# bmds-lab/Crackling

Measured on AMD Instinct MI355X. Metric: guides/sec (whole node) + achieved HBM GB/s, 20bp/<=4mm ISSL scan, higher is better.
Workload: dtype u32

## Files before the change

### crackling_amd/csrc/issl_device.hpp

```cpp
#pragma once
#include <cstddef>
#include <cstdint>
#include <string>

#include "issl_host.hpp"

namespace issl {

constexpr uint64_t kImageMagic = 0x314C535349444D41ull;
constexpr uint32_t kImageVersion = 9;
constexpr uint32_t kTileCands = 2048;
constexpr uint32_t kHeaderBytes = 4096;

struct ImageHeader {
    uint64_t magic;
    uint32_t version;
    uint32_t kind;
    uint64_t n_sites, seq_len, n_lines, slice_width, n_slices, n_scores_file;
    uint64_t n_buckets;
    uint64_t n_scores_unique;
    uint64_t n_tiles;
    uint64_t tile_cands;
    uint64_t total_bytes;
    uint64_t off_bucket_start, off_tile_first, off_score_mask, off_score_val, off_sites, off_entries,
        off_scan;
    uint64_t off_mit_dense;
    uint64_t off_esig;
    uint64_t cold_on_host;
    uint64_t cold_bytes;
    uint64_t off_occ8;
    uint64_t off_sub_start;
    uint64_t off_srec;
    uint64_t off_sid;
    uint64_t off_site_occ;
    uint64_t lists_absent;
};
static_assert(sizeof(ImageHeader) <= kHeaderBytes, "header must fit its block");

constexpr uint32_t kOccSaturated = 0xFFFFFFu;
constexpr uint64_t kSigMask = (1ull << 40) - 1ull;

#if defined(__HIPCC__)
__host__ __device__
#endif
inline uint32_t succ_byte(uint64_t sig, uint32_t s, uint32_t slice_width)
{
    const uint32_t sh = (slice_width * (s + 1u)) % 40u;
    const uint64_t x = sig & kSigMask;
    return static_cast<uint32_t>(sh ? (x >> sh) | (x << (40u - sh)) : x) & 0xFFu;
}
struct alignas(16) StreamRec {
    uint64_t sig;
    uint32_t id;
    uint32_t pos;
};

struct ImageView {
    const uint64_t *bucket_start;
    const uint32_t *tile_first;
    const uint64_t *score_mask;
    const double *score_val;
    const double *mit_dense;
    const uint64_t *sites;
    const uint64_t *entries;
    const uint64_t *esig;
    const uint8_t *occ8;
    const uint32_t *sub_start;
    const StreamRec *srec;
    const uint32_t *sid;
    const uint32_t *site_occ;
    const uint32_t *scan;
    uint64_t n_sites;
    uint32_t n_buckets;
    uint32_t n_scores;
    uint32_t slice_width;
    uint32_t n_slices;
    uint32_t n_tiles;
};

struct LayoutSpec {
    bool inline_sigs = false;
    uint32_t cold = 0;
    uint32_t sorted = 0;
    bool no_lists = false;
};
void layout_image(ImageHeader &h, const Geometry &g, uint64_t n_scores_unique, uint64_t n_tiles, bool dense_mit,
                  const LayoutSpec &spec);
ImageView make_view(const ImageHeader &h, void *base, void *cold);

struct Tuning {
    uint32_t scan_blocks;
    uint32_t scan_threads;
    int upload_threads;
    size_t upload_chunk_kib, upload_ring_min_kib;
    uint32_t item_guides;
    bool scan_generic;
    int scan_events;
    bool stage_timing;
    bool upload_timing;
    size_t raw_chunks;
    int inline_sigs;
    int sorted_layout;
    int compact;
    int prune;
    int tail_shapes;
    int hit_slots;
    size_t fine_items;
    size_t expect_guides;
    int small_bin;
    int lean_tail;
    int lanes;
    int host_cold;
    int keep_lists;
    std::string stamps_path;
    static Tuning from_env();
    bool set(const char *key, const char *value);
    bool get(const char *key, long long *value) const;
    int set_list(const char *options);
};
bool image_option(const ImageHeader *h, const char *key, long long *value);

int launch_build_entries(const uint64_t *d_sites, const uint32_t *d_occ, uint64_t n_sites, uint32_t slice_begin,
                         uint32_t slice_end, uint32_t slice_width, uint64_t *d_entries);
int launch_bucket_sizes(const uint64_t *d_sites, uint64_t n_sites, uint32_t slice_width, uint32_t n_slices, uint64_t *h_sizes);

constexpr int kSortNeedsListOrder = -1000;
constexpr int kSortNoRoom = -1001;
struct SortTemp {
    uint64_t *keys = nullptr, *tmp = nullptr;
    uint32_t *hist = nullptr;
    bool keys_borrowed = false;
    int alloc(uint64_t n_sites, void *borrowed_keys = nullptr);
    void release();
    ~SortTemp() { release(); }
};
int launch_sort_slice(SortTemp &t, const uint64_t *d_sites, const uint64_t *d_list, const uint64_t *d_bucket_start,
                      const uint32_t *d_tile_first, uint64_t n_sites, uint32_t n_slices, uint32_t n_buckets, uint32_t slice_width, uint32_t slice, uint32_t *d_sub_start,
                      StreamRec *d_srec, uint32_t *d_sid, uint32_t *d_site_occ, uint32_t *d_flag);
int finish_sort(uint32_t *d_flag);
void launch_tag_sites(uint64_t *d_sites, const uint32_t *d_site_occ, uint64_t n_sites);

constexpr uint32_t kGuideGroup = 8;
constexpr uint32_t kItemGuides = 512;
constexpr uint32_t kGuideCost = 4;
constexpr uint32_t kTileFixedCost = 8 * kGuideCost;
constexpr uint32_t kNoGuide = 0xFFFFFFFFu;
constexpr uint32_t kPadGuideWord = 0xFFFFFFFFu;
constexpr uint32_t kScanGridBlocks = 256u * 4u;
constexpr uint32_t kScanMaxBlocks = 8192u;
constexpr uint32_t kScanWaves = kScanMaxBlocks * 16u;
constexpr uint32_t kMaxRanges = kScanMaxBlocks;
constexpr uint32_t kStampsScanWords = 4u * kScanWaves, kStampsPerReplay = 16u * 4096u;
constexpr uint32_t kStampsMid = kStampsScanWords, kStampsBig256 = kStampsMid + kStampsPerReplay, kStampsBig1024 = kStampsBig256 + kStampsPerReplay;
constexpr uint32_t kStampsWords = kStampsBig1024 + kStampsPerReplay;
constexpr uint32_t kSpanRing = 64;
constexpr uint32_t kChunkRecs = 128;
constexpr uint64_t kDeadKey = ~0ull;
constexpr uint32_t kKeySliceShift = 32, kKeyGuideShift = 37, kKeySliceMask = 31, kMaxSlices = 20;

struct ScanItem {
    uint32_t bucket;
    uint32_t g0, g1;
    uint32_t n_tiles;
    uint64_t cost0;
    uint32_t tile0;
    uint32_t last_cands;
    uint32_t group_abs;
    uint32_t window;
    uint32_t shape;
    uint32_t gmid;
};
static_assert(sizeof(ScanItem) == 48, "scan items are fetched with scalar loads");

struct RangeStart {
    uint32_t item;
    uint32_t tile;
    uint32_t goff;
    uint32_t pad;
};

struct PlanInfo {
    uint32_t n_items;
    uint32_t error;
    uint32_t n_ranges;
    uint32_t fine;
    uint64_t total_cost;
    uint64_t candidates;
    uint64_t reference_candidates;
    uint64_t tiles;
    uint32_t fine_slots;
    uint32_t pad;
};

struct Counters {
    uint32_t next_range;
    uint32_t n_big;
    uint32_t n_big2;
    uint32_t n_big3;
    uint32_t raw_chunks;
    uint32_t raw_overflow;
    uint32_t overflowed;
    uint32_t replay_next[3];
};

struct FineSum {
    uint64_t cost, cand;
    uint32_t slots, items, units;
    uint32_t places;
};

constexpr uint32_t kSlotHits = 512;
constexpr uint32_t kSlotHitsWide = 2048;
struct alignas(32) SlotRec {
    double mit, cfd;
    uint64_t key, pad;
};
#if defined(__HIPCC__)
__host__ __device__
#endif
inline uint64_t slot_pad(uint32_t occ, uint32_t dist) { return static_cast<uint64_t>(occ) | (static_cast<uint64_t>(dist) << 32); }
constexpr uint32_t kFineWays = 13;
constexpr uint32_t kFineWays2 = 67;
constexpr uint32_t kFetchPairs = 8;
constexpr uint32_t kPruneMaxGuides = 1u << 20;
constexpr uint32_t kPruneMaxGuides2 = 1u << 18;
inline uint32_t prune_max_guides(uint32_t prune_mode, uint32_t n_slices)
{
    const uint32_t m = prune_mode == 3 ? kPruneMaxGuides2 : kPruneMaxGuides;
    return n_slices > 10 ? m >> 2 : n_slices > 5 ? m >> 1 : m;
}

struct alignas(16) FineMeta {
    uint32_t guide;
    uint32_t where;
    uint64_t gsig;
};

struct Workspace {
    uint32_t *ng = nullptr;
    uint32_t *gfill = nullptr;
    uint32_t *gstart = nullptr;
    uint32_t *gword = nullptr;
    uint32_t *gidx = nullptr;
    uint32_t *gbucket = nullptr;
    ScanItem *items = nullptr;
    uint32_t *fword = nullptr;
    FineMeta *fmeta = nullptr;
    ScanItem *fitems = nullptr;
    uint32_t *fcount = nullptr;
    uint32_t *fcount0 = nullptr;
    FineSum *fsum = nullptr;
    size_t cap_fslots = 0, cap_fitems = 0;
    uint32_t fine_ways = 0;
    PlanInfo *plan = nullptr;
    RangeStart *range_start = nullptr;
    uint64_t *raw = nullptr;
    uint32_t *raw_used = nullptr;
    size_t cap_chunks = 0;
    Counters *counters = nullptr;
    unsigned long long *scan_span = nullptr;
    uint32_t span_slot = 0;
    uint64_t *scan_count = nullptr;
// ... 59 lines not shown
```

### crackling_amd/csrc/issl_kernels.hip

```cpp
#include <hip/hip_runtime.h>

#include <algorithm>
#include <type_traits>
#include <cstdio>

#include "issl_device.hpp"

namespace issl {

#define ISSL_CFD_QUAL __constant__
#include "cfd_tables.inc"


__device__ __forceinline__ void short_kernel_priority() { __builtin_amdgcn_s_setprio(3); }

__host__ __device__ inline uint32_t gather_even16(uint32_t x)
{
    x &= 0x55555555u;
    x = (x | (x >> 1)) & 0x33333333u;
    x = (x | (x >> 2)) & 0x0F0F0F0Fu;
    x = (x | (x >> 4)) & 0x00FF00FFu;
    x = (x | (x >> 8)) & 0x0000FFFFu;
    return x;
}
// ... 405 lines not shown
           (u.rest ? static_cast<uint64_t>(len) * (u.shape >> 3) + kTileFixedCost : 0ull);
}

__device__ __forceinline__ uint32_t fine_way(uint32_t gj, uint32_t way)
{
    if (way == 0) return gj;
    if (way < kFineWays) {
        const uint32_t q = (way - 1u) / 3u, d = (way - 1u) % 3u + 1u;
        return gj ^ (d << (2u * q));
    }
    const uint32_t w2 = way - kFineWays, pair = w2 / 9u, d1 = (w2 % 9u) / 3u + 1u, d2 = w2 % 3u + 1u;
    const uint32_t a = pair < 3u ? 0u : pair < 5u ? 1u : 2u;
    const uint32_t b = pair < 3u ? pair + 1u : pair < 5u ? pair - 1u : 3u;
    return gj ^ (d1 << (2u * a)) ^ (d2 << (2u * b));
}
__device__ __forceinline__ uint32_t fine_class(uint32_t way) { return way == 0u ? 0u : way < kFineWays ? 1u : 2u; }

__host__ __device__ __forceinline__ uint32_t fine_quad(uint32_t slice) { return slice < 4u ? slice : 0u; }
__host__ __device__ __forceinline__ uint32_t fine_order(uint32_t slice, uint32_t j, uint32_t slice_width = 8u)
{
    if (slice_width != 8u) return j + 1u;
    const uint32_t sq = fine_quad(slice);
    if (slice == 0u) return j + 1u;
    const uint32_t prev = slice - 1u;
    if (j == 0u) return prev;
    uint32_t q = 0, seen = 0;
    for (; q < 4u; ++q) {
        if (q == sq || q == prev) continue;
        if (++seen == j) break;
    }
    return q;
}
__host__ __device__ __forceinline__ uint32_t fine_word(uint32_t word, uint32_t slice, uint32_t slice_width = 8u)
{
    const uint32_t lo = word & 0xFFFFu, hi = word >> 16;
    uint32_t lo12 = 0, hi12 = 0;
    for (uint32_t j = 0; j < 3u; ++j) {
        const uint32_t q = fine_order(slice, j, slice_width);
        lo12 |= ((lo >> (4u * q)) & 0xFu) << (4u * j);
        hi12 |= ((hi >> (4u * q)) & 0xFu) << (4u * j);
    }
    return lo12 | (hi12 << 12);
}

template <uint32_t WAYS>
__global__ __launch_bounds__(256) void k_fine_count(ImageView v, const uint64_t *__restrict__ guides,
                                                    const uint32_t *__restrict__ gstart, const uint32_t *__restrict__ gfill,
                                                    const uint32_t *__restrict__ gidx, uint32_t *__restrict__ fcount,
                                                    uint32_t *__restrict__ fcount0,
                                                    FineSum *__restrict__ fsum, uint32_t item_guides, uint32_t tail_shapes)
{
    constexpr uint32_t ways = WAYS;
    short_kernel_priority();
    __shared__ uint32_t cnt[256], cnt0[256];
    __shared__ uint64_t lds[256];
    const uint32_t b = blockIdx.x, slice = b >> v.slice_width;
    cnt[threadIdx.x] = 0;
    cnt0[threadIdx.x] = 0;
    __syncthreads();
    const uint32_t g0 = gstart[b], n = gfill[b];
    for (uint32_t i = threadIdx.x; i < n; i += 256) {
        const uint32_t gj = succ_byte(guides[gidx[g0 + i]], slice, v.slice_width);
        atomicAdd(&cnt0[gj], 1u);
#pragma unroll
        for (uint32_t way = 0; way < ways; ++way) atomicAdd(&cnt[fine_way(gj, way)], 1u);
    }
    __syncthreads();
    const uint32_t w = threadIdx.x, c = cnt[w];
    const uint32_t *ss = v.sub_start + static_cast<uint64_t>(b) * 257u;
    const uint32_t s0 = ss[w], s1 = ss[w + 1];
    fcount[static_cast<uint64_t>(b) * 256u + w] = (s1 > s0) ? c : 0u;
    fcount0[static_cast<uint64_t>(b) * 256u + w] = (s1 > s0) ? cnt0[w] : 0u;
    uint64_t cost = 0, cand = 0, slots = 0, items = 0, units = 0;
    if (c && s1 > s0) {
        const GroupUnits gu = group_units(s0, s1, tail_shapes);
        const uint32_t kk = (c + item_guides - 1u) / item_guides;
        slots = (c + kGuideGroup - 1u) / kGuideGroup * kGuideGroup;
        units = static_cast<uint64_t>(gu.units) * kk;
        items = units;
        for (uint32_t done = 0; done < c; done += item_guides) cost += group_cost(gu, c - done < item_guides ? c - done : item_guides);
        cand = static_cast<uint64_t>(s1 - s0) * c;
    }
    uint64_t t_cost, t_cand, t_slots, t_items, t_units, t_places;
    (void)block_exclusive_scan(cost, lds, &t_cost);
    (void)block_exclusive_scan(cand, lds, &t_cand);
    (void)block_exclusive_scan(slots, lds, &t_slots);
    (void)block_exclusive_scan(items, lds, &t_items);
    (void)block_exclusive_scan(units, lds, &t_units);
    (void)block_exclusive_scan((c && s1 > s0) ? c : 0u, lds, &t_places);
    if (threadIdx.x == 0) {
        FineSum f;
        f.cost = t_cost; f.cand = t_cand; f.slots = static_cast<uint32_t>(t_slots); f.items = static_cast<uint32_t>(t_items);
        f.units = static_cast<uint32_t>(t_units); f.places = static_cast<uint32_t>(t_places);
        fsum[b] = f;
    }
}

__global__ __launch_bounds__(256) void k_fine_plan(FineSum *__restrict__ fsum, uint32_t nb, ScanItem *__restrict__ fitems,
                                                   uint32_t cap_items, uint32_t cap_slots, PlanInfo *__restrict__ plan,
                                                   uint32_t scan_blocks, uint32_t prune_mode, uint32_t always,
                                                   uint32_t *__restrict__ sticky, Counters *__restrict__ counters)
{
    short_kernel_priority();
    __shared__ uint64_t lds[256];
    const uint32_t per = (nb + 255u) / 256u;
    const uint32_t b0 = threadIdx.x * per, b1 = (b0 + per < nb) ? b0 + per : nb;
    uint64_t cost = 0, cand = 0, slots = 0, items = 0, units = 0, places = 0;
    for (uint32_t b = b0; b < b1; ++b) {
        cost += fsum[b].cost; cand += fsum[b].cand; slots += fsum[b].slots; items += fsum[b].items; units += fsum[b].units;
        places += fsum[b].places;
    }
    uint64_t t_cost, t_cand, t_slots, t_items, t_units, t_places;
    (void)block_exclusive_scan(places, lds, &t_places);
    uint64_t cost_at = block_exclusive_scan(cost, lds, &t_cost);
    (void)block_exclusive_scan(cand, lds, &t_cand);
    uint64_t slot_at = block_exclusive_scan(slots, lds, &t_slots);
    uint64_t item_at = block_exclusive_scan(items, lds, &t_items);
    uint64_t unit_at = block_exclusive_scan(units, lds, &t_units);
    for (uint32_t b = b0; b < b1; ++b) {
        const FineSum f = fsum[b];
        FineSum at;
        at.cost = cost_at; at.cand = 0; at.slots = static_cast<uint32_t>(slot_at); at.items = static_cast<uint32_t>(item_at);
        at.units = static_cast<uint32_t>(unit_at); at.places = 0;
        fsum[b] = at;
        cost_at += f.cost; slot_at += f.slots; item_at += f.items; unit_at += f.units;
    }
    if (threadIdx.x == 255) {
        const uint64_t fetch_cost = static_cast<uint64_t>(kFetchPairs) * kGuideCost;
        const uint64_t full_fetch = plan->tiles, full_pairs = plan->total_cost - kTileFixedCost * full_fetch;
        const uint64_t fine_pairs = t_cost - kTileFixedCost * t_units;
        const uint64_t est_full = full_pairs > fetch_cost * full_fetch ? full_pairs : fetch_cost * full_fetch;
        const uint64_t est_fine = (fine_pairs > fetch_cost * t_units ? fine_pairs : fetch_cost * t_units) + t_places * kGuideCost;
        const bool fits = t_items <= cap_items && t_slots <= cap_slots;
        if (t_items > cap_items)
            atomicMax(&sticky[3], static_cast<uint32_t>(t_items < 0xFFFFFFFFull ? t_items : 0xFFFFFFFFull));
        if (fits && plan->error == 0 && (always || est_fine < est_full)) {
            ScanItem end;
            end.bucket = 0; end.g0 = 0; end.g1 = 0; end.n_tiles = 0; end.cost0 = t_cost;
            end.tile0 = static_cast<uint32_t>(t_units); end.last_cands = 0; end.group_abs = 0; end.window = 0;
            end.shape = 32; end.gmid = 0;
            fitems[t_items] = end;
            plan->n_items = static_cast<uint32_t>(t_items);
            plan->total_cost = t_cost;
            plan->candidates = t_cand;
            plan->tiles = t_units;
            plan->n_ranges = t_units == 0 ? 0u : ranges_for(t_units, scan_blocks);
            counters->raw_chunks = (plan->n_ranges ? plan->n_ranges : 1u) * 16u;
            plan->fine = prune_mode;
            plan->fine_slots = static_cast<uint32_t>(t_slots);
        }
    }
}

template <uint32_t WAYS>
__global__ __launch_bounds__(256) void k_fine_scatter(ImageView v, const uint64_t *__restrict__ guides,
                                                      const uint32_t *__restrict__ gstart, const uint32_t *__restrict__ gfill,
                                                      const uint32_t *__restrict__ gword, const uint32_t *__restrict__ gidx,
                                                      const uint32_t *__restrict__ fcount, const uint32_t *__restrict__ fcount0,
                                                      const FineSum *__restrict__ fbase,
                                                      const PlanInfo *__restrict__ plan, uint32_t *__restrict__ fword,
                                                      FineMeta *__restrict__ fmeta,
                                                      ScanItem *__restrict__ fitems, uint32_t item_guides, uint32_t tail_shapes)
{
    constexpr uint32_t ways = WAYS;
    short_kernel_priority();
    if (!plan->fine) return;
    __shared__ uint64_t lds[256];
    __shared__ uint32_t slot_of[256], slot0_of[256], cursor[256], cursor0[256], has_cands[256];
    const uint32_t b = blockIdx.x, slice = b >> v.slice_width;
    const uint32_t w = threadIdx.x;
    const uint32_t c = fcount[static_cast<uint64_t>(b) * 256u + w];
    const uint32_t c1 = c - fcount0[static_cast<uint64_t>(b) * 256u + w];
    const uint32_t *ss = v.sub_start + static_cast<uint64_t>(b) * 257u;
    const uint32_t s0 = ss[w], s1 = ss[w + 1];
    uint64_t cost = 0, slots = 0, items = 0;
    uint32_t kk = 0;
    GroupUnits gu{};
    if (c) {
        gu = group_units(s0, s1, tail_shapes);
        kk = (c + item_guides - 1u) / item_guides;
        slots = (c + kGuideGroup - 1u) / kGuideGroup * kGuideGroup;
        items = static_cast<uint64_t>(gu.units) * kk;
        for (uint32_t done = 0; done < c; done += item_guides) cost += group_cost(gu, c - done < item_guides ? c - done : item_guides);
    }
    const FineSum base = fbase[b];
    uint64_t cost_at = base.cost + block_exclusive_scan(cost, lds, nullptr);
    const uint32_t slot_at = base.slots + static_cast<uint32_t>(block_exclusive_scan(slots, lds, nullptr));
    uint32_t item_at = base.items + static_cast<uint32_t>(block_exclusive_scan(items, lds, nullptr));
    slot_of[w] = slot_at;
    slot0_of[w] = slot_at + c1;
    cursor[w] = 0;
    cursor0[w] = 0;
    __shared__ uint32_t item0_of[257], c_of[256];
    __shared__ uint64_t cost0_of[256];
    __shared__ __attribute__((aligned(16))) ScanItem stage[256];
    item0_of[w] = item_at - base.items;
    if (w == 255u) item0_of[256] = item_at - base.items + static_cast<uint32_t>(items);
    c_of[w] = c;
    cost0_of[w] = cost_at;
    if (c)
        for (uint32_t k2 = c; k2 < static_cast<uint32_t>(slots); ++k2) { fmeta[slot_at + k2] = FineMeta{kNoGuide, 0u, 0ull}; fword[slot_at + k2] = kPadGuideWord; }
    has_cands[w] = s1 > s0 ? 1u : 0u;
    __syncthreads();
    {
        const uint32_t total = item0_of[256];
        const uint64_t blen = v.bucket_start[b + 1] - v.bucket_start[b];
        const uint32_t tile_first_b = v.tile_first[b];
        for (uint32_t i0 = 0; i0 < total; i0 += 256u) {
            const uint32_t i = i0 + w;
            if (i < total) {
                uint32_t lo = 0, hi = 256;
                while (hi - lo > 1u) {
                    const uint32_t mid = (lo + hi) >> 1;
                    if (item0_of[mid] <= i) lo = mid; else hi = mid;
                }
                const uint32_t gw = lo, gc = c_of[gw];
                const uint32_t gs0 = ss[gw], gs1 = ss[gw + 1];
                const GroupUnits g2 = group_units(gs0, gs1, tail_shapes);
                const uint32_t j = i - item0_of[gw];
                const uint32_t chunk = j / g2.units, t = j - chunk * g2.units;
                const uint32_t done = chunk * item_guides;
                const uint32_t len = (gc - done < item_guides) ? gc - done : item_guides;
                const bool full = t < g2.n_full;
                const uint32_t shape = full ? 32u : g2.shape, cap = 64u * shape;
                const uint32_t wstart = g2.s0a + t * kTileCands;
                const uint64_t after = blen - wstart;
                const uint32_t gslot = slot_of[gw];
                ScanItem it;
                it.bucket = (b << 8) | gw;
                it.g0 = gslot + done;
                it.g1 = it.g0 + len;
                it.n_tiles = 1;
                it.cost0 = cost0_of[gw] + static_cast<uint64_t>(chunk) * group_cost(g2, item_guides) +
                           static_cast<uint64_t>(t) * (static_cast<uint64_t>(len) * kGuideCost + kTileFixedCost);
                it.tile0 = base.items + i;
                it.last_cands = after < cap ? static_cast<uint32_t>(after) : cap;
                it.group_abs = tile_first_b * 64u + (wstart >> 5);
                it.window = (t == 0 ? gs0 - g2.s0a : 0u) | ((gs1 - wstart < cap ? gs1 - wstart : cap) << 16);
                it.shape = shape; it.gmid = slot0_of[gw];
                stage[w] = it;
            }
            __syncthreads();
            const uint32_t n_here = total - i0 < 256u ? total - i0 : 256u;
            const uint4 *src4 = reinterpret_cast<const uint4 *>(stage);
            uint4 *dst4 = reinterpret_cast<uint4 *>(fitems + base.items + i0);
            for (uint32_t q = w; q < n_here * 3u; q += 256u) dst4[q] = src4[q];
            __syncthreads();
        }
    }
    const uint32_t g0 = gstart[b], n = gfill[b];
    for (uint32_t i = threadIdx.x; i < n; i += 256) {
        const uint32_t guide = gidx[g0 + i], word = gword[g0 + i];
        const uint64_t gsig = guides[guide];
        const uint32_t gj = succ_byte(gsig, slice, v.slice_width);
        const uint32_t word12 = fine_word(word, slice, v.slice_width);
#pragma unroll
        for (uint32_t way = 0; way < ways; ++way) {
            const uint32_t ww = fine_way(gj, way);
            if (!has_cands[ww]) continue;
            const uint32_t slot = way ? slot_of[ww] + atomicAdd(&cursor[ww], 1u) : slot0_of[ww] + atomicAdd(&cursor0[ww], 1u);
            fword[slot] = word12 | (fine_class(way) << 24);
            fmeta[slot] = FineMeta{guide, (b << 8) | ww, gsig};
        }
    }
}

__global__ __launch_bounds__(256) void k_fine_ranges(const PlanInfo *__restrict__ plan, const ScanItem *__restrict__ fitems,
                                                     RangeStart *__restrict__ starts)
{
    short_kernel_priority();
    if (!plan->fine) return;
    const uint32_t n_ranges = plan->n_ranges;
    const uint32_t r = blockIdx.x * 4u + (threadIdx.x >> 6);
    if (r <= n_ranges && n_ranges != 0) {
        const RangeStart st = range_start_of<true>(fitems, plan->n_items, plan->total_cost, n_ranges, r);
        if ((threadIdx.x & 63u) == 0u) starts[r] = st;
    }
}

constexpr uint32_t kSmallPairs = 512;

__device__ inline uint64_t block512_exclusive_scan(uint64_t v, uint64_t *lds , uint64_t *total)
{
    const uint32_t lane = threadIdx.x & 63u, wave = threadIdx.x >> 6;
    const uint64_t incl = wave_inclusive_scan_u64(v);
    if (lane == 63) lds[wave] = incl;
    __syncthreads();
    uint64_t before = 0, all = 0;
    for (uint32_t w = 0; w < kSmallPairs / 64u; ++w) {
        const uint64_t x = lds[w];
        if (w < wave) before += x;
        all += x;
    }
    if (total) *total = all;
    __syncthreads();
    return before + incl - v;
}

template <uint32_t WAYS>
__global__ __launch_bounds__(kSmallPairs) void k_bin_small(ImageView v, Workspace ws, const uint64_t *__restrict__ guides, uint32_t n,
                                                           uint32_t prune_mode, uint32_t tail_shapes, uint32_t scan_blocks,
                                                           uint32_t sorted_layout)
{
    short_kernel_priority();
    __shared__ uint64_t lds[kSmallPairs / 64u];
    const uint32_t t = threadIdx.x, my_way = blockIdx.x;
    for (uint32_t k = my_way * kSmallPairs + t; k <= n; k += WAYS * kSmallPairs) ws.gcount[k] = 0;
    for (uint32_t k = my_way * kSmallPairs + t; k <= ws.cap_chunks; k += WAYS * kSmallPairs) ws.raw_used[k] = 0;
    if (t == 0 && my_way == 0) {
        ws.scan_span[2u * ws.span_slot] = ~0ull;
        ws.scan_span[2u * ws.span_slot + 1u] = 0ull;
    }
    const uint32_t pairs = n * v.n_slices;
    const uint32_t low = (1u << v.slice_width) - 1u;
    const bool mine = t < pairs;
    const uint32_t g = mine ? t / v.n_slices : 0u, sl = mine ? t - g * v.n_slices : 0u;
    uint64_t sig = 0, blen = 0, units = 0, cost = 0, cand = 0, ref = 0, valid = 0;
    uint64_t cost_before = 0;
    uint32_t units_before = 0, valid_before = 0;
    uint32_t b = 0, gj = 0, tf = 0, my_s0 = 0, my_s1 = 0;
    if (mine) {
        sig = guides[g];
        b = (sl << v.slice_width) + (static_cast<uint32_t>(sig >> (v.slice_width * sl)) & low);
        gj = succ_byte(sig, sl, v.slice_width);
        const uint32_t *ss = v.sub_start + static_cast<uint64_t>(b) * 257u;
        uint32_t s0[WAYS], s1[WAYS];
#pragma unroll
        for (uint32_t way = 0; way < WAYS; ++way) {
            const uint32_t ww = fine_way(gj, way);
            s0[way] = ss[ww];
            s1[way] = ss[ww + 1];
        }
        blen = v.bucket_start[b + 1] - v.bucket_start[b];
        tf = v.tile_first[b];
        ref = blen;
#pragma unroll
        for (uint32_t way = 0; way < WAYS; ++way) {
            if (way == my_way) { my_s0 = s0[way]; my_s1 = s1[way]; units_before = static_cast<uint32_t>(units); cost_before = cost; valid_before = static_cast<uint32_t>(valid); }
            if (s1[way] > s0[way]) {
                const GroupUnits gu = group_units(s0[way], s1[way], tail_shapes);
                units += gu.units;
                cost += group_cost(gu, 1u);
                cand += s1[way] - s0[way];
                ++valid;
            }
        }
    }
    uint64_t t_units, t_cost, t_cand, t_ref, t_valid;
    uint32_t item_at = static_cast<uint32_t>(block512_exclusive_scan(units, lds, &t_units)) + units_before;
    uint64_t cost_at = block512_exclusive_scan(cost, lds, &t_cost) + cost_before;
    (void)block512_exclusive_scan(cand, lds, &t_cand);
    (void)block512_exclusive_scan(ref, lds, &t_ref);
    const uint32_t slot_at = (static_cast<uint32_t>(block512_exclusive_scan(valid, lds, &t_valid)) + valid_before) * kGuideGroup;
    const uint64_t t_slots = t_valid * kGuideGroup;
    const bool overflow = t_units > ws.cap_fitems || t_slots > ws.cap_fslots;
    if (mine && !overflow && my_s1 > my_s0) {
        const uint32_t way = my_way, s0 = my_s0, s1 = my_s1;
        const uint32_t word12 = fine_word(image_word(sig, sl, v.slice_width, sorted_layout != 0u), sl, v.slice_width);
        const uint32_t ww = fine_way(gj, way);
        const uint32_t c1 = way ? 1u : 0u;
        uint4 *fw = reinterpret_cast<uint4 *>(ws.fword + slot_at);
        fw[0] = make_uint4(word12 | (fine_class(way) << 24), kPadGuideWord, kPadGuideWord, kPadGuideWord);
        fw[1] = make_uint4(kPadGuideWord, kPadGuideWord, kPadGuideWord, kPadGuideWord);
        ws.fmeta[slot_at] = FineMeta{g, (b << 8) | ww, sig};
#pragma unroll
        for (uint32_t k2 = 1; k2 < kGuideGroup; ++k2) ws.fmeta[slot_at + k2] = FineMeta{kNoGuide, 0u, 0ull};
        const GroupUnits gu = group_units(s0, s1, tail_shapes);
        for (uint32_t u = 0; u < gu.units; ++u) {
            const bool full = u < gu.n_full;
            const uint32_t shape = full ? 32u : gu.shape, cap = 64u * shape;
            const uint32_t wstart = gu.s0a + u * kTileCands;
            const uint64_t after = blen - wstart;
            ScanItem it;
            it.bucket = (b << 8) | ww;
            it.g0 = slot_at;
            it.g1 = slot_at + 1u;
            it.n_tiles = 1;
            it.cost0 = cost_at;
            it.tile0 = item_at;
            it.last_cands = after < cap ? static_cast<uint32_t>(after) : cap;
            it.group_abs = tf * 64u + (wstart >> 5);
            it.window = (u == 0 ? s0 - gu.s0a : 0u) | ((s1 - wstart < cap ? s1 - wstart : cap) << 16);
            it.shape = shape; it.gmid = slot_at + c1;
            ws.fitems[item_at++] = it;
            cost_at += static_cast<uint64_t>(shape >> 3) + kTileFixedCost;
        }
    }
    if (t == 0 && my_way == 0) {
        const uint32_t n_items = overflow ? 0u : static_cast<uint32_t>(t_units);
        ScanItem end;
        end.bucket = 0; end.g0 = 0; end.g1 = 0; end.n_tiles = 0; end.cost0 = overflow ? 0ull : t_cost;
        end.tile0 = n_items; end.last_cands = 0; end.group_abs = 0; end.window = 0; end.shape = 32; end.gmid = 0;
        ws.fitems[n_items] = end;
        PlanInfo pl{};
        pl.n_items = n_items;
        pl.error = 0;
        pl.n_ranges = n_items == 0 ? 0u : ranges_for(t_units, scan_blocks);
        pl.fine = prune_mode;
        pl.total_cost = overflow ? 0ull : t_cost;
        pl.candidates = overflow ? 0ull : t_cand;
        pl.reference_candidates = t_ref;
        pl.tiles = n_items;
        pl.fine_slots = overflow ? 0u : static_cast<uint32_t>(t_slots);
        *ws.plan = pl;
        Counters c{};
        c.raw_chunks = (pl.n_ranges ? pl.n_ranges : 1u) * 16u;
        *ws.counters = c;
        if (overflow) {
            atomicMax(&ws.sticky[3], static_cast<uint32_t>(t_units < 0xFFFFFFFFull ? t_units : 0xFFFFFFFFull));
            atomicOr(&ws.sticky[0], 2u);
        }
    }
}

static bool small_bin_ok(const ImageView &v, const Workspace &ws, const Tuning &tn, uint32_t n, uint32_t prune_mode)
{
    if (!tn.small_bin || (prune_mode != 1u && prune_mode != 2u) || !ws.fitems || !v.sub_start) return false;
    if (n == 0 || static_cast<uint64_t>(n) * v.n_slices > kSmallPairs) return false;
    const uint64_t buckets_per_slice = 1ull << v.slice_width;
    return tn.prune == 1 || v.n_sites / buckets_per_slice >= 16ull * kTileCands;
}

uint32_t prune_mode_for(const ImageView &v, const Tuning &tn, uint32_t n_guides, int max_dist)
{
    const bool geometry = v.n_slices * v.slice_width == 40u && (v.slice_width == 8 || v.slice_width == 4 || v.slice_width == 2);
    if ((!v.srec && !v.sid) || tn.prune == 0 || max_dist < 0 || max_dist > 5 || !geometry) return 0;
    if (n_guides > prune_max_guides(max_dist == 5 ? 3u : 2u, v.n_slices)) return 0;
    return max_dist <= 2 ? 1u : max_dist <= 4 ? 2u : 3u;
}

void launch_bin_guides(const ImageView &v, const Workspace &ws, const Tuning &tn, const uint64_t *d_guides, uint32_t n,
                       uint32_t prune_mode, void *stream_)
{
    hipStream_t stream = static_cast<hipStream_t>(stream_);
    const uint32_t nb = v.n_buckets;
    if (small_bin_ok(v, ws, tn, n, prune_mode)) {
        const uint32_t sorted = (v.srec || v.sid) ? 1u : 0u;
        if (fine_ways_of(prune_mode) == 1u)
            hipLaunchKernelGGL(k_bin_small<1u>, dim3(1), dim3(kSmallPairs), 0, stream, v, ws, d_guides, n, prune_mode,
                               static_cast<uint32_t>(tn.tail_shapes), tn.scan_blocks, sorted);
        else
            hipLaunchKernelGGL(k_bin_small<kFineWays>, dim3(kFineWays), dim3(kSmallPairs), 0, stream, v, ws, d_guides, n, prune_mode,
                               static_cast<uint32_t>(tn.tail_shapes), tn.scan_blocks, sorted);
        hipLaunchKernelGGL(k_fine_ranges, dim3((tn.scan_blocks + 1u + 3u) / 4u), dim3(256), 0, stream, ws.plan, ws.fitems, ws.range_start);
        return;
    }
    const uint32_t n_slots = static_cast<uint32_t>(
        std::min<size_t>(ws.cap_gslots, static_cast<size_t>(n) * v.n_slices + static_cast<size_t>(kGuideGroup) * nb));
    const uint32_t blocks = (n + 255u) / 256u;
    const uint32_t reset_blocks = std::min<uint32_t>(1024u, (std::max(n_slots, nb) + 255u) / 256u);
    hipLaunchKernelGGL(k_guide_hist, dim3(std::max(blocks, reset_blocks)), dim3(256), 0, stream, ws, d_guides, n,
                       v.slice_width, v.n_slices, nb, n_slots, tn.scan_blocks * 16u);
    hipLaunchKernelGGL(k_plan, dim3(1), dim3(256), 0, stream, v, ws.ng, ws.gfill, ws.gstart, ws.items,
                       static_cast<uint32_t>(ws.cap_items), ws.plan, tn.item_guides, tn.scan_blocks, ws.counters);
    const uint32_t range_blocks = (tn.scan_blocks + 1u + 255u) / 256u;
    hipLaunchKernelGGL(k_guide_scatter, dim3(blocks + range_blocks), dim3(256), 0, stream, d_guides, n, v.slice_width,
                       v.n_slices, (v.srec || v.sid) ? 1u : 0u, nb, ws.gstart, ws.gfill, ws.gword, ws.gidx, ws.gbucket, blocks, ws.plan, ws.items,
                       ws.range_start);
    if (prune_mode) {
        const uint32_t ways = fine_ways_of(prune_mode);
        const uint32_t tail_shapes = prune_mode == 3 ? 0u : static_cast<uint32_t>(tn.tail_shapes);
        auto launch_fine = [&](auto ways_tag) {
            constexpr uint32_t W = decltype(ways_tag)::value;
            hipLaunchKernelGGL(k_fine_count<W>, dim3(nb), dim3(256), 0, stream, v, d_guides, ws.gstart, ws.gfill, ws.gidx, ws.fcount,
                               ws.fcount0, ws.fsum, tn.item_guides, tail_shapes);
            hipLaunchKernelGGL(k_fine_plan, dim3(1), dim3(256), 0, stream, ws.fsum, nb, ws.fitems,
                               static_cast<uint32_t>(ws.cap_fitems), static_cast<uint32_t>(ws.cap_fslots), ws.plan, tn.scan_blocks,
                               prune_mode, tn.prune == 1 ? 1u : 0u, ws.sticky, ws.counters);
            hipLaunchKernelGGL(k_fine_scatter<W>, dim3(nb), dim3(256), 0, stream, v, d_guides, ws.gstart, ws.gfill, ws.gword, ws.gidx,
                               ws.fcount, ws.fcount0, ws.fsum, ws.plan, ws.fword, ws.fmeta, ws.fitems, tn.item_guides, tail_shapes);
        };
        if (ways == 1u) launch_fine(std::integral_constant<uint32_t, 1u>{});
        else if (ways == kFineWays) launch_fine(std::integral_constant<uint32_t, kFineWays>{});
        else launch_fine(std::integral_constant<uint32_t, kFineWays2>{});
        hipLaunchKernelGGL(k_fine_ranges, dim3((tn.scan_blocks + 1u + 3u) / 4u), dim3(256), 0, stream, ws.plan, ws.fitems, ws.range_start);
    }
}


struct alignas(4 * kGuideGroup) GuideGroup {
    uint32_t w[kGuideGroup];
};


__device__ __forceinline__ uint64_t raw_record(uint32_t gslot, uint32_t tile, uint32_t offset)
{
    return (static_cast<uint64_t>(gslot) << 37) | (static_cast<uint64_t>(tile) << 11) | offset;
}

struct RawWriter {
    uint64_t *chunk;
    uint32_t fill;
    uint32_t left;
    uint32_t reserve;
};

__device__ __forceinline__ void raw_retire(const RawWriter &w, uint32_t lane, const uint64_t *raw, uint32_t *raw_used)
{
    if (lane == 0) raw_used[(w.chunk - raw) / kChunkRecs] = w.fill;
}

__device__ __forceinline__ void raw_acquire(RawWriter &w, uint64_t *raw, uint32_t max_chunks, Counters *counters,
                                            uint32_t lane)
{
    w.fill = 1;
    if (w.left != 0u) {
        w.chunk += kChunkRecs;
        w.left -= 1u;
        return;
    }
    const uint32_t take = w.reserve;
    uint32_t idx = 0;
    if (lane == 0) idx = atomicAdd(&counters->raw_chunks, take);
    idx = __builtin_amdgcn_readfirstlane(idx);
    if (idx + take > max_chunks) {
        idx = max_chunks;
        if (lane == 0) counters->raw_overflow = 1u;
        w.chunk = raw + static_cast<uint64_t>(idx) * kChunkRecs;
        return;
    }
    w.chunk = raw + static_cast<uint64_t>(idx) * kChunkRecs;
    w.left = take - 1u;
    if (take < 16u) w.reserve = take * 2u;
}

__device__ __forceinline__ void full_add(uint32_t a, uint32_t b, uint32_t c, uint32_t &sum, uint32_t &carry)
{
    sum = __builtin_amdgcn_bitop3_b32(a, b, c, 0x96);
    carry = __builtin_amdgcn_bitop3_b32(a, b, c, 0xE8);
}
__device__ __forceinline__ void half_add(uint32_t a, uint32_t b, uint32_t &sum, uint32_t &carry)
{
    sum = a ^ b;
    carry = a & b;
}

template <int THR>
__device__ __forceinline__ uint32_t count_near(const uint32_t (&m)[16], uint32_t thr, uint32_t keep);

template <int THR>
__device__ __forceinline__ uint32_t near_plane(const uint32_t (&c)[kPlanes], uint32_t gw, uint32_t thr, uint32_t keep)
{
    uint32_t m[16];
#pragma unroll
    for (int p = 0; p < 16; ++p) {
        const uint32_t g0 = 0u - ((gw >> p) & 1u);
        const uint32_t g1 = 0u - ((gw >> (16 + p)) & 1u);
        m[p] = (c[p] ^ g0) | (c[16 + p] ^ g1);
    }
    return count_near<THR>(m, thr, keep);
}

template <int THR>
__device__ __forceinline__ uint32_t near_plane_masks(const uint32_t (&c)[kPlanes], const uint4 *gm ,
                                                     uint32_t thr, uint32_t keep)
{
    uint32_t m[16];
#pragma unroll
    for (int q = 0; q < 4; ++q) {
        const uint4 lo = gm[q], hi = gm[4 + q];
        asm volatile("" ::: "memory");
        m[4 * q + 0] = (c[4 * q + 0] ^ lo.x) | (c[16 + 4 * q + 0] ^ hi.x);
        m[4 * q + 1] = (c[4 * q + 1] ^ lo.y) | (c[16 + 4 * q + 1] ^ hi.y);
        m[4 * q + 2] = (c[4 * q + 2] ^ lo.z) | (c[16 + 4 * q + 2] ^ hi.z);
        m[4 * q + 3] = (c[4 * q + 3] ^ lo.w) | (c[16 + 4 * q + 3] ^ hi.w);
    }
    return count_near<THR>(m, thr, keep);
}

__device__ __forceinline__ void short_unit_masks(const uint32_t *__restrict__ gword_stream, uint32_t g0, uint32_t shape,
                                                 uint32_t lane, uint4 *lds_masks)
{
    const uint32_t per = 32u / shape, field = shape == 16u ? 0xFFFFu : 0xFFu;
    const uint32_t i = lane >> 3, q = lane & 7u;
    uint32_t gw[4];
#pragma unroll
    for (uint32_t j = 0; j < 4; ++j) gw[j] = j < per ? gword_stream[g0 + i * per + j] : 0u;
    uint32_t m[4];
#pragma unroll
    for (uint32_t r = 0; r < 4; ++r) {
        const uint32_t p = 4u * q + r;
        uint32_t x = 0;
#pragma unroll
        for (uint32_t j = 0; j < 4; ++j) x |= (0u - ((gw[j] >> p) & 1u)) & (field << ((j * shape) & 31u)) & (j < per ? ~0u : 0u);
        m[r] = x;
    }
    lds_masks[i * 8u + q] = make_uint4(m[0], m[1], m[2], m[3]);
}

template <int THR>
__device__ __forceinline__ uint32_t count_near(const uint32_t (&m)[16], uint32_t thr, uint32_t keep)
{
    uint32_t s0, s1, s2, s3, s4, t, u, n0, n1, n2;
    uint32_t k2[8], k4[4], k8a, k8b;
    full_add(m[0], m[1], m[2], s0, k2[0]);
    full_add(m[3], m[4], m[5], s1, k2[1]);
    full_add(m[6], m[7], m[8], s2, k2[2]);
    full_add(m[9], m[10], m[11], s3, k2[3]);
    full_add(m[12], m[13], m[14], s4, k2[4]);
    full_add(s0, s1, s2, t, k2[5]);
    full_add(s3, s4, m[15], u, k2[6]);
    half_add(t, u, n0, k2[7]);
    uint32_t a2, b2, c2;
    full_add(k2[0], k2[1], k2[2], a2, k4[0]);
    full_add(k2[3], k2[4], k2[5], b2, k4[1]);
    full_add(k2[6], k2[7], a2, c2, k4[2]);
    half_add(b2, c2, n1, k4[3]);
    if (THR >= 0 && THR <= 4) {
        const uint32_t o = __builtin_amdgcn_bitop3_b32(k4[0], k4[1], k4[2], 0xFE);
        if (THR == 0) return __builtin_amdgcn_bitop3_b32(o, __builtin_amdgcn_bitop3_b32(k4[3], n1, n0, 0xFE), keep, 0x02);
        if (THR == 1) return __builtin_amdgcn_bitop3_b32(o, k4[3], n1, 0x01) & keep;
        if (THR == 2) return __builtin_amdgcn_bitop3_b32(o, __builtin_amdgcn_bitop3_b32(k4[3], n1, n0, 0xF8), keep, 0x02);
        if (THR == 3) return __builtin_amdgcn_bitop3_b32(o, k4[3], keep, 0x02);
        const uint32_t p = __builtin_amdgcn_bitop3_b32(k4[0], k4[1], k4[2], 0xE8);
        const uint32_t z = __builtin_amdgcn_bitop3_b32(o, k4[3], n1 | n0, 0xE8);
        return __builtin_amdgcn_bitop3_b32(p, z, keep, 0x02);
    }
    uint32_t a4;
    full_add(k4[0], k4[1], k4[2], a4, k8a);
    half_add(a4, k4[3], n2, k8b);
    const uint32_t n[5] = {n0, n1, n2, k8a ^ k8b, k8a & k8b};
    uint32_t gt = 0u, eq = ~0u;
#pragma unroll
// ... 1815 lines not shown
```

### crackling_amd/csrc/issl_options.cpp

```cpp
#include <climits>
#include <cstdlib>
#include <cstring>
#include <string>

#include "issl_device.hpp"

namespace issl {

namespace {

enum Kind { kInt, kFlag, kTri, kPath };

template <class T, T Tuning::*M> void put(Tuning &t, long long v) { t.*M = static_cast<T>(v); }
template <class T, T Tuning::*M> long long get(const Tuning &t) { return static_cast<long long>(t.*M); }
#define MEMBER(m) put<decltype(Tuning::m), &Tuning::m>, get<decltype(Tuning::m), &Tuning::m>

struct Option {
    const char *key, *env;
    Kind kind;
    long long lo, hi, def;
    void (*put)(Tuning &, long long);
    long long (*get)(const Tuning &);
    long long multiple = 1;
    long long round = 1;
};

constexpr long long kNoMax = LLONG_MAX;

const Option kOptions[] = {
    {"scan_blocks", "ISSL_SCAN_BLOCKS", kInt, 1, kScanMaxBlocks, kScanGridBlocks, MEMBER(scan_blocks)},
    {"scan_threads", "ISSL_SCAN_THREADS", kInt, 64, 1024, 1024, MEMBER(scan_threads), 64},
    {"upload_chunk_kib", "ISSL_UPLOAD_CHUNK_KIB", kInt, 4, 1 << 20, 16384, MEMBER(upload_chunk_kib)},
    {"upload_ring_min_kib", "ISSL_UPLOAD_RING_MIN_KIB", kInt, 0, kNoMax, 65536, MEMBER(upload_ring_min_kib)},
    {"upload_threads", "ISSL_UPLOAD_THREADS", kInt, 1, 32, 8, MEMBER(upload_threads)},
    {"item_guides", "ISSL_ITEM_GUIDES", kInt, 8, kItemGuides, kItemGuides, MEMBER(item_guides), 1, 8},
    {"scan_generic", "ISSL_SCAN_GENERIC", kFlag, 0, 1, 0, MEMBER(scan_generic)},
    {"stage_timing", "ISSL_STAGE_TIMING", kFlag, 0, 1, 0, MEMBER(stage_timing)},
    {"scan_events", "ISSL_SCAN_EVENTS", kInt, 0, 2, 2, MEMBER(scan_events)},
    {"raw_chunks", "ISSL_RAW_CHUNKS", kInt, 0, kNoMax, 0, MEMBER(raw_chunks)},
    {"inline_sigs", "ISSL_INLINE_SIGS", kTri, -1, 1, -1, MEMBER(inline_sigs)},
    {"host_cold", "ISSL_FORCE_HOST_COLD", kTri, -1, 1, -1, MEMBER(host_cold)},
    {"scan_stamps", "ISSL_SCAN_STAMPS", kPath, 0, 0, 0, nullptr, nullptr},
    {"sorted_layout", "ISSL_SORTED_LAYOUT", kTri, -1, 1, -1, MEMBER(sorted_layout)},
    {"prune", "ISSL_PRUNE", kTri, -1, 1, -1, MEMBER(prune)},
    {"lanes", "ISSL_LANES", kInt, 1, 3, 1, MEMBER(lanes)},
    {"compact", "ISSL_COMPACT", kTri, -1, 1, -1, MEMBER(compact)},
    {"tail_shapes", "ISSL_TAIL_SHAPES", kFlag, 0, 1, 1, MEMBER(tail_shapes)},
    {"hit_slots", "ISSL_HIT_SLOTS", kInt, 0, 2, 1, MEMBER(hit_slots)},
    {"lean_tail", "ISSL_LEAN_TAIL", kFlag, 0, 1, 1, MEMBER(lean_tail)},
    {"small_bin", "ISSL_SMALL_BIN", kFlag, 0, 1, 1, MEMBER(small_bin)},
    {"expect_guides", "ISSL_EXPECT_GUIDES", kInt, 0, kNoMax, 0, MEMBER(expect_guides)},
    {"fine_items", "ISSL_FINE_ITEMS", kInt, 0, kNoMax, 0, MEMBER(fine_items)},
    {"keep_lists", "ISSL_KEEP_LISTS", kTri, -1, 1, -1, MEMBER(keep_lists)},
};
#undef MEMBER

const Option *find(const char *key)
{
    for (const Option &o : kOptions)
        if (std::strcmp(o.key, key) == 0) return &o;
    return nullptr;
}

struct ImageKey {
    const char *key;
    long long (*get)(const ImageHeader &h);
};

const ImageKey kImageKeys[] = {
    {"is_sorted", [](const ImageHeader &h) -> long long { return (h.off_srec || h.off_sid) ? 1 : 0; }},
    {"is_compact", [](const ImageHeader &h) -> long long { return h.off_sid ? 1 : 0; }},
    {"cold_on_host", [](const ImageHeader &h) -> long long { return h.cold_on_host ? 1 : 0; }},
    {"cold_sections", [](const ImageHeader &h) -> long long { return h.cold_on_host; }},
    {"lists_absent", [](const ImageHeader &h) -> long long { return h.lists_absent; }},
    {"dense_mit", [](const ImageHeader &h) -> long long { return h.off_mit_dense ? 1 : 0; }},
    {"has_inline_sigs", [](const ImageHeader &h) -> long long { return h.off_esig ? 1 : 0; }},
};

}

Tuning Tuning::from_env()
{
    Tuning t;
    for (const Option &o : kOptions)
        if (o.put) o.put(t, o.def);
    const char *timing = std::getenv("ISSL_UPLOAD_TIMING");
    t.upload_timing = timing && timing[0] == '1';
    for (const Option &o : kOptions)
        if (const char *e = std::getenv(o.env)) (void)t.set(o.key, e);
    return t;
}

bool Tuning::set(const char *key, const char *value)
{
    const Option *o = key && value ? find(key) : nullptr;
    if (!o) return false;
    if (o->kind == kPath) {
        stamps_path = value;
        return true;
    }
    char *end = nullptr;
    const long long n = std::strtoll(value, &end, 10);
    if (end == value || *end != 0 || n < o->lo || n > o->hi || n % o->multiple) return false;
    o->put(*this, n / o->round * o->round);
    return true;
}

bool Tuning::get(const char *key, long long *value) const
{
    const Option *o = find(key);
    if (!o || o->kind == kPath) return false;
    *value = o->get(*this);
    return true;
}

int Tuning::set_list(const char *options)
{
    for (std::string rest = options ? options : ""; !rest.empty();) {
        const size_t comma = rest.find(',');
        const std::string item = rest.substr(0, comma);
        rest = comma == std::string::npos ? std::string() : rest.substr(comma + 1);
        const size_t eq = item.find('=');
        if (eq == std::string::npos || !set(item.substr(0, eq).c_str(), item.substr(eq + 1).c_str())) {
            set_error("unknown option or value out of range: " + item);
            return ISSL_E_ARG;
        }
    }
    return ISSL_OK;
}

bool image_option(const ImageHeader *h, const char *key, long long *value)
{
    for (const ImageKey &k : kImageKeys)
        if (std::strcmp(k.key, key) == 0) {
            *value = h ? k.get(*h) : -1;
            return true;
        }
    return false;
}

}
```

Baseline: 43.28 million.

## Stage fine-scatter slot writes in LDS windows and flush them coalesced

In k_fine_scatter, the per-bucket fine slots (FineMeta and the fine word) are now assembled in an LDS image covering up to 16 windows of slot ranges. Each window is then copied to global memory with vectorized uint4 stores, replacing the scattered per-guide atomic-indexed global writes. Guide loads for the first two strides are held in registers, so repeated passes over the windows reuse them. In exchange the kernel loops over the guides once per window and adds block syncs and much more LDS, which can lower occupancy. Large buckets and sub-buckets that overflow a window still take the direct-write path.

```diff
diff --git a/crackling_amd/csrc/issl_device.hpp b/crackling_amd/csrc/issl_device.hpp
--- a/crackling_amd/csrc/issl_device.hpp
+++ b/crackling_amd/csrc/issl_device.hpp
@@ -108,6 +108,7 @@
     size_t fine_items;
     size_t expect_guides;
     int small_bin;
+    bool stage_slots;
     int lean_tail;
     int lanes;
     int host_cold;
diff --git a/crackling_amd/csrc/issl_kernels.hip b/crackling_amd/csrc/issl_kernels.hip
--- a/crackling_amd/csrc/issl_kernels.hip
+++ b/crackling_amd/csrc/issl_kernels.hip
@@ -581,6 +581,13 @@
     }
 }
 
+constexpr uint32_t kStageSlots = 1536;
+constexpr uint32_t kStageStride = 1280;
+constexpr uint32_t kStageWindows = 16;
+constexpr uint32_t kStageHeld = 2;
+constexpr uint32_t kModeDirect = 0xFFu, kModeNone = 0xFEu;
+static_assert(kStageSlots * 20u >= 256u * sizeof(ScanItem) && kStageStride % 8u == 0 && kStageStride < kStageSlots, "k_fine_scatter's image");
+
 template <uint32_t WAYS>
 __global__ __launch_bounds__(256) void k_fine_scatter(ImageView v, const uint64_t *__restrict__ guides,
                                                       const uint32_t *__restrict__ gstart, const uint32_t *__restrict__ gfill,
@@ -589,15 +596,18 @@
                                                       const FineSum *__restrict__ fbase,
                                                       const PlanInfo *__restrict__ plan, uint32_t *__restrict__ fword,
                                                       FineMeta *__restrict__ fmeta,
-                                                      ScanItem *__restrict__ fitems, uint32_t item_guides, uint32_t tail_shapes)
+                                                      ScanItem *__restrict__ fitems, uint32_t item_guides, uint32_t tail_shapes,
+                                                      uint32_t staged)
 {
     constexpr uint32_t ways = WAYS;
     short_kernel_priority();
     if (!plan->fine) return;
     __shared__ uint64_t lds[256];
-    __shared__ uint32_t slot_of[256], slot0_of[256], cursor[256], cursor0[256], has_cands[256];
+    __shared__ uint32_t slot_of[256], slot0_of[256], cursor[256], cursor0[256], mode[256];
+    __shared__ uint32_t win_lo[kStageWindows], win_hi[kStageWindows];
     const uint32_t b = blockIdx.x, slice = b >> v.slice_width;
     const uint32_t w = threadIdx.x;
+    if (w < kStageWindows) { win_lo[w] = ~0u; win_hi[w] = 0u; }
     const uint32_t c = fcount[static_cast<uint64_t>(b) * 256u + w];
     const uint32_t c1 = c - fcount0[static_cast<uint64_t>(b) * 256u + w];
     const uint32_t *ss = v.sub_start + static_cast<uint64_t>(b) * 257u;
@@ -614,22 +624,37 @@
     }
     const FineSum base = fbase[b];
     uint64_t cost_at = base.cost + block_exclusive_scan(cost, lds, nullptr);
-    const uint32_t slot_at = base.slots + static_cast<uint32_t>(block_exclusive_scan(slots, lds, nullptr));
+    uint64_t tot_slots;
+    const uint32_t off = static_cast<uint32_t>(block_exclusive_scan(slots, lds, &tot_slots));
+    const uint32_t slot_at = base.slots + off;
     uint32_t item_at = base.items + static_cast<uint32_t>(block_exclusive_scan(items, lds, nullptr));
+    const bool stage_bucket = staged && tot_slots <= static_cast<uint64_t>(kStageStride) * kStageWindows;
+    const uint32_t n_win = stage_bucket ? (static_cast<uint32_t>(tot_slots) + kStageStride - 1u) / kStageStride : 0u;
+    const uint32_t win = off / kStageStride;
+    if (c && stage_bucket) atomicMin(&win_lo[win], off);
     slot_of[w] = slot_at;
     slot0_of[w] = slot_at + c1;
     cursor[w] = 0;
     cursor0[w] = 0;
     __shared__ uint32_t item0_of[257], c_of[256];
     __shared__ uint64_t cost0_of[256];
-    __shared__ __attribute__((aligned(16))) ScanItem stage[256];
+    __shared__ __attribute__((aligned(16))) uint8_t image[kStageSlots * 20u];
+    ScanItem *stage = reinterpret_cast<ScanItem *>(image);
+    FineMeta *m_img = reinterpret_cast<FineMeta *>(image);
+    uint32_t *w_img = reinterpret_cast<uint32_t *>(image + kStageSlots * 16u);
     item0_of[w] = item_at - base.items;
     if (w == 255u) item0_of[256] = item_at - base.items + static_cast<uint32_t>(items);
     c_of[w] = c;
     cost0_of[w] = cost_at;
-    if (c)
+    __syncthreads();
+    uint32_t my_mode = s1 > s0 ? kModeDirect : kModeNone;
+    if (c && stage_bucket && off + static_cast<uint32_t>(slots) <= win_lo[win] + kStageSlots) {
+        my_mode = win;
+        atomicMax(&win_hi[win], off + static_cast<uint32_t>(slots));
+    }
+    mode[w] = my_mode;
+    if (c && my_mode == kModeDirect)
         for (uint32_t k2 = c; k2 < static_cast<uint32_t>(slots); ++k2) { fmeta[slot_at + k2] = FineMeta{kNoGuide, 0u, 0ull}; fword[slot_at + k2] = kPadGuideWord; }
-    has_cands[w] = s1 > s0 ? 1u : 0u;
     __syncthreads();
     {
         const uint32_t total = item0_of[256];
@@ -678,19 +703,55 @@
         }
     }
     const uint32_t g0 = gstart[b], n = gfill[b];
-    for (uint32_t i = threadIdx.x; i < n; i += 256) {
-        const uint32_t guide = gidx[g0 + i], word = gword[g0 + i];
-        const uint64_t gsig = guides[guide];
-        const uint32_t gj = succ_byte(gsig, slice, v.slice_width);
-        const uint32_t word12 = fine_word(word, slice, v.slice_width);
-#pragma unroll
-        for (uint32_t way = 0; way < ways; ++way) {
-            const uint32_t ww = fine_way(gj, way);
-            if (!has_cands[ww]) continue;
-            const uint32_t slot = way ? slot_of[ww] + atomicAdd(&cursor[ww], 1u) : slot0_of[ww] + atomicAdd(&cursor0[ww], 1u);
-            fword[slot] = word12 | (fine_class(way) << 24);
-            fmeta[slot] = FineMeta{guide, (b << 8) | ww, gsig};
-        }
+    uint32_t held_guide[kStageHeld], held_word[kStageHeld];
+    uint64_t held_sig[kStageHeld];
+#pragma unroll
+    for (uint32_t j = 0; j < kStageHeld; ++j) {
+        const uint32_t i = w + 256u * j;
+        held_guide[j] = i < n ? gidx[g0 + i] : 0u;
+        held_word[j] = i < n ? gword[g0 + i] : 0u;
+    }
+#pragma unroll
+    for (uint32_t j = 0; j < kStageHeld; ++j) held_sig[j] = w + 256u * j < n ? guides[held_guide[j]] : 0ull;
+    for (uint32_t k = 0; k < (n_win ? n_win : 1u); ++k) {
+        const uint32_t lo = win_lo[k], hi = win_hi[k];
+        const uint32_t img0 = base.slots + lo;
+        if (c && my_mode == k)
+            for (uint32_t k2 = c; k2 < static_cast<uint32_t>(slots); ++k2) { m_img[off - lo + k2] = FineMeta{kNoGuide, 0u, 0ull}; w_img[off - lo + k2] = kPadGuideWord; }
+        for (uint32_t i = w, j = 0; i < n; i += 256u, ++j) {
+            uint32_t guide, word;
+            uint64_t gsig;
+            if (j < kStageHeld) {
+                guide = j ? held_guide[kStageHeld - 1u] : held_guide[0];
+                word = j ? held_word[kStageHeld - 1u] : held_word[0];
+                gsig = j ? held_sig[kStageHeld - 1u] : held_sig[0];
+            } else {
+                guide = gidx[g0 + i]; word = gword[g0 + i];
+                gsig = guides[guide];
+            }
+            const uint32_t gj = succ_byte(gsig, slice, v.slice_width);
+            const uint32_t word12 = fine_word(word, slice, v.slice_width);
+#pragma unroll
+            for (uint32_t way = 0; way < ways; ++way) {
+                const uint32_t ww = fine_way(gj, way);
+                const uint32_t m = mode[ww];
+                if (m != k && !(m == kModeDirect && k == 0u)) continue;
+                const uint32_t slot = way ? slot_of[ww] + atomicAdd(&cursor[ww], 1u) : slot0_of[ww] + atomicAdd(&cursor0[ww], 1u);
+                const uint32_t fw = word12 | (fine_class(way) << 24);
+                const FineMeta fm{guide, (b << 8) | ww, gsig};
+                if (m == k) { w_img[slot - img0] = fw; m_img[slot - img0] = fm; }
+                else { fword[slot] = fw; fmeta[slot] = fm; }
+            }
+        }
+        __syncthreads();
+        if (hi > lo) {
+            const uint32_t n_out = hi - lo;
+            const uint4 *ms = reinterpret_cast<const uint4 *>(m_img), *wsrc = reinterpret_cast<const uint4 *>(w_img);
+            uint4 *md = reinterpret_cast<uint4 *>(fmeta + img0), *wd = reinterpret_cast<uint4 *>(fword + img0);
+            for (uint32_t q = w; q < n_out; q += 256u) md[q] = ms[q];
+            for (uint32_t q = w; q < n_out / 4u; q += 256u) wd[q] = wsrc[q];
+        }
+        __syncthreads();
     }
 }
 
@@ -897,7 +958,8 @@
                                static_cast<uint32_t>(ws.cap_fitems), static_cast<uint32_t>(ws.cap_fslots), ws.plan, tn.scan_blocks,
                                prune_mode, tn.prune == 1 ? 1u : 0u, ws.sticky, ws.counters);
             hipLaunchKernelGGL(k_fine_scatter<W>, dim3(nb), dim3(256), 0, stream, v, d_guides, ws.gstart, ws.gfill, ws.gword, ws.gidx,
-                               ws.fcount, ws.fcount0, ws.fsum, ws.plan, ws.fword, ws.fmeta, ws.fitems, tn.item_guides, tail_shapes);
+                               ws.fcount, ws.fcount0, ws.fsum, ws.plan, ws.fword, ws.fmeta, ws.fitems, tn.item_guides, tail_shapes,
+                               tn.stage_slots ? 1u : 0u);
         };
         if (ways == 1u) launch_fine(std::integral_constant<uint32_t, 1u>{});
         else if (ways == kFineWays) launch_fine(std::integral_constant<uint32_t, kFineWays>{});
diff --git a/crackling_amd/csrc/issl_options.cpp b/crackling_amd/csrc/issl_options.cpp
--- a/crackling_amd/csrc/issl_options.cpp
+++ b/crackling_amd/csrc/issl_options.cpp
@@ -86,6 +86,8 @@
         if (o.put) o.put(t, o.def);
     const char *timing = std::getenv("ISSL_UPLOAD_TIMING");
     t.upload_timing = timing && timing[0] == '1';
+    const char *stage = std::getenv("ISSL_STAGE_SLOTS");
+    t.stage_slots = !(stage && stage[0] == '0');
     for (const Option &o : kOptions)
         if (const char *e = std::getenv(o.env)) (void)t.set(o.key, e);
     return t;
```

Result: no change. 43.61 million (median of 6 runs) (+0.8%).
